# homenc/HElib

Hardware: AMD Instinct MI355X
Metric: ctxt_x_ctxt_mults_per_sec_incl_relinearize (higher is better)
Workload: dtype u64; 1 GPU; BGV m=32768 p=65537 bits=950 (L=16x60b, K=6x56b, 6 small primes, D=3): Ctxt::multiplyBy on FRESH ciphertexts = multLowLvl (bringToSet x2 + tensorProduct) + reLinearize (dropSmallAndSpecialPrimes + key switch), benchmarks/bgv_basic.cpp:144-165; added noise MEASURED as in the reference (device canonical-embedding norms, read back lazily); the loop is driven by the C++17 host (libhelib_amd_host.so); ; batch_per_gpu=128, pairs_all_ranks=128

## Files before the change

### helib_amd/build.py

```python
import os
import shutil
import subprocess
import sys
from concurrent.futures import ThreadPoolExecutor

HERE = os.path.dirname(os.path.abspath(__file__))
CSRC = os.path.join(HERE, "csrc")
LIBDIR = os.path.join(HERE, "lib")
SO = os.path.join(LIBDIR, "libhelib_amd.so")
UNITS = [("ntt_kernels.hip", ["-DHX_NTT_ONLY=13", "-DHX_NTT_PART=1"], "ntt_kernels_13.o"),
         ("ntt_kernels.hip", ["-DHX_NTT_ONLY=14", "-DHX_NTT_PART=1"], "ntt_kernels_14.o"),
         ("ntt_kernels.hip", ["-DHX_NTT_ONLY=15", "-DHX_NTT_PART=1"], "ntt_kernels_15.o"),
         ("ntt_kernels.hip", ["-DHX_NTT_ONLY=13", "-DHX_NTT_PART=2"], "ntt_kslast_13.o"),
         ("ntt_kernels.hip", ["-DHX_NTT_ONLY=14", "-DHX_NTT_PART=2"], "ntt_kslast_14.o"),
         ("ntt_kernels.hip", ["-DHX_NTT_ONLY=15", "-DHX_NTT_PART=2"], "ntt_kslast_15.o"), ("ntt_dispatch.hip", [], "ntt_dispatch.o"),
         ("conv_kernels.hip", [], "conv_kernels.o"), ("pfa_kernels.hip", [], "pfa_kernels.o"), ("rns_mfma_kernels.hip", [], "rns_mfma_kernels.o"),
         ("ckks_slots.hip", [], "ckks_slots.o"), ("bgv_slots.hip", [], "bgv_slots.o"), ("bgv_crt.hip", [], "bgv_crt.o"),
         ("bgv_gf.hip", [], "bgv_gf.o"), ("bgv_gf_linalg.hip", [], "bgv_gf_linalg.o"),
         ("linalg.hip", [], "linalg.o"),
         ("engine.hip", [], "engine.o")]
SOURCES = sorted({u[0] for u in UNITS})
HEADERS = ["ntt_core.h", "dev_common.h", "rns_kernels.h", "rns_types.h", "hostmath.h", "conv_core.h", "bluestein.h", "norm_kernels.h",
           "prg_kernels.h", "arena.h", "prof.h", "conv_dev.h", "ntt_kernel_util.h", "norm_r16.h", "fft_lds.h", "work_map.h",
           os.path.join("..", "..", "include", "helib_amd.h")]
UNIT_HEADERS = {"pfa_kernels.hip": ["pfa_core.h", "pfa_dev.h"], "rns_mfma_kernels.hip": ["mfma_ext.h", "rns_mfma_dev.h"],
                "engine.hip": ["pfa_core.h", "pfa_dev.h", "switches.h", "mfma_ext.h", "rns_mfma_dev.h", "ckks_bridge.h"],
                "ckks_slots.hip": ["ckks_slots.h", "ckks_bridge.h"], "bgv_slots.hip": ["bgv_slots.h", "bgv_encode.h", "ckks_bridge.h"],
                "bgv_crt.hip": ["bgv_slots.h", "bgv_encode.h", "bgv_crt.h", "ckks_bridge.h"],
                "bgv_gf.hip": ["bgv_slots.h", "bgv_encode.h", "bgv_crt.h", "bgv_gf.h", "bgv_gf_tail.h", "ckks_bridge.h"],
                "bgv_gf_linalg.hip": ["bgv_slots.h", "bgv_encode.h", "bgv_crt.h", "bgv_gf.h", "bgv_gf_linalg.h", "bgv_gf_tail.h",
                                      "gather_map.h", "ckks_bridge.h"],
                "linalg.hip": ["ckks_bridge.h"]}
FLAGS = ["--offload-arch=gfx950", "-O3", "-std=c++17", "-fPIC", "-Wno-unused-value",
         "-Wno-pass-failed"]


def hipcc():
    for cand in (shutil.which("hipcc"), "/opt/rocm/bin/hipcc"):
        if cand and os.path.exists(cand):
            return cand
    raise RuntimeError("hipcc not found: the MI355X engine cannot be built")


def _stale(target, deps):
    if not os.path.exists(target):
        return True
    t = os.path.getmtime(target)
    return any(os.path.getmtime(d) > t for d in deps if os.path.exists(d))


def build(force=False, extra_flags=(), verbose=False):
    os.makedirs(LIBDIR, exist_ok=True)
    deps = [os.path.join(CSRC, h) for h in HEADERS] + [os.path.abspath(__file__)]
    cc = hipcc()
    objs, jobs = [], []
    for s, unit_flags, o in UNITS:
        src = os.path.join(CSRC, s)
        obj = os.path.join(LIBDIR, o)
        objs.append(obj)
        if force or _stale(obj, deps + [src] + [os.path.join(CSRC, h) for h in UNIT_HEADERS.get(s, [])]):
            jobs.append([cc, *FLAGS, *unit_flags, *extra_flags, "-c", src, "-o", obj])

    def run(cmd):
        if verbose:
            print(" ".join(cmd), file=sys.stderr)
        subprocess.check_call(cmd)

    if jobs:
        with ThreadPoolExecutor(max_workers=len(jobs)) as ex:
            list(ex.map(run, jobs))
    if jobs or force or _stale(SO, objs):
        run([cc, "--offload-arch=gfx950", "-shared", "-fPIC", "-o", SO, *objs])
    build_host(force=force, verbose=verbose)
    return SO


HOST_SO = os.path.join(LIBDIR, "libhelib_amd_host.so")


def build_host(force=False, verbose=False, link_dir=None, link_lib="helib_amd", out=None):
    inc = os.path.join(HERE, "..", "include")
    src = os.path.join(CSRC, "host_session.cpp")
    out = out or HOST_SO
    deps = [src] + [os.path.join(inc, h) for h in os.listdir(inc)]
    if not (force or _stale(out, deps)):
        return out
    cmd = ["g++", "-std=c++17", "-O2", "-fPIC", "-shared", "-Wall", "-I" + inc, src, "-L" + (link_dir or LIBDIR),
           "-l" + link_lib, "-Wl,-rpath," + (link_dir or "$ORIGIN"), "-o", out]
    if verbose:
        print(" ".join(cmd), file=sys.stderr)
    subprocess.check_call(cmd)
    return out


if __name__ == "__main__":
    print(build(force="--force" in sys.argv, verbose=True))
```

### helib_amd/csrc/dev_common.h

```cpp
#pragma once
#include <hip/hip_runtime.h>
#include <stdint.h>

#include "ntt_core.h"

namespace hx {

constexpr int MAX_ROWS = 160;

struct PrimeDev {
  uint64_t q;
  uint64_t q2;
  uint64_t mu;
  uint64_t mu64;
  uint32_t k;
  uint32_t proth;
  uint64_t mu63;
  uint64_t tw_fwd_off;
  uint64_t tw_inv_off;
  uint64_t r2;
  uint64_t half_t1, half_t1p, half_t1m;
};

struct RowMap {
// ... 49 lines not shown
}
__device__ __forceinline__ uint64_t ld_stream1(const uint64_t* p)
{
#if defined(HX_NO_NT) || defined(HX_RNS_NO_NT)
  return *p;
#else
  return __builtin_nontemporal_load(p);
#endif
}
__device__ __forceinline__ void st_stream1(uint64_t* p, uint64_t v)
{
#if defined(HX_NO_NT) || defined(HX_RNS_NO_NT)
  *p = v;
#else
  __builtin_nontemporal_store(v, p);
#endif
}
__device__ __forceinline__ void st_stream2(uint64_t* p, ulonglong2 v)
{
#ifdef HX_NO_NT
  *reinterpret_cast<ulonglong2*>(p) = v;
#else
  hx_v2u64 w;
  w.x = v.x;
  w.y = v.y;
  __builtin_nontemporal_store(w, reinterpret_cast<hx_v2u64*>(p));
#endif
}
#endif

struct TensorSrc {
  const uint64_t* a0;
  const uint64_t* a1;
  const uint64_t* b0;
  const uint64_t* b1;
};
constexpr int MD_MAXPOLY = 8;
struct PolyBases {
  uint64_t* d[MD_MAXPOLY];
  int n;
};
__host__ __device__ inline uint64_t* poly_base(const PolyBases& p, unsigned i)
{
  uint64_t* r = p.d[0];
  r = i == 1 ? p.d[1] : r;
  r = i == 2 ? p.d[2] : r;
  r = i == 3 ? p.d[3] : r;
  r = i == 4 ? p.d[4] : r;
  r = i == 5 ? p.d[5] : r;
  r = i == 6 ? p.d[6] : r;
  r = i == 7 ? p.d[7] : r;
  return r;
}
struct RowMap2 {
  uint16_t p[MAX_ROWS];
  uint16_t brow[MAX_ROWS];
};
struct RowScalars {
  uint64_t c[MAX_ROWS];
  uint64_t cp[MAX_ROWS];
};

constexpr int KS_MAXD = 8;
struct KsFix {
  int64_t owner;
  TW pinv[KS_MAXD];
  TW pscale;
};
struct KsLastPlan {
  uint16_t fd[MAX_ROWS];
};
struct KsLastArgs {
  const uint64_t* dig_in;
  const uint64_t* dig_ev;
  const uint64_t* kb;
  const uint64_t* ka;
  uint64_t* out0;
  uint64_t* out1;
  const uint64_t* own_src;
  const uint64_t* acc0;
  const uint64_t* acc1;
  const KsFix* fix;
  int nall, wrows, batch, scale_parts;
};

typedef unsigned __int128 u128;

#define HX_RO __attribute__((address_space(4)))
typedef const HX_RO uint64_t* ro_u64;
typedef const HX_RO uint32_t* ro_u32;
typedef const HX_RO double* ro_f64;
typedef const HX_RO TW* ro_tw;
template <class T>
__host__ __device__ inline const HX_RO T* as_ro(const T* p)
{
  return (const HX_RO T*)(uintptr_t)p;
}
__device__ __forceinline__ TW ld_tw(ro_tw p, size_t i)
{
  ro_u64 w = (ro_u64)p;
  TW t;
  t.w = w[2 * i];
  t.wp = w[2 * i + 1];
  return t;
}

__device__ __forceinline__ uint64_t add_mod(uint64_t a, uint64_t b, uint64_t q)
{
  uint64_t s = a + b;
  return s >= q ? s - q : s;
}
__device__ __forceinline__ uint64_t sub_mod(uint64_t a, uint64_t b, uint64_t q)
{
  return a >= b ? a - b : a + q - b;
}
__device__ __forceinline__ uint64_t neg_mod(uint64_t a, uint64_t q) { return a ? q - a : 0; }

__device__ __forceinline__ uint64_t mul_mod(uint64_t a, uint64_t b, uint64_t q, uint64_t mu,
                                            uint32_t k)
{
  u128 x = (u128)a * b;
  uint64_t xs = (uint64_t)(x >> (k - 1));
  uint64_t qh = (uint64_t)(((u128)xs * mu) >> (k + 1));
  uint64_t r = (uint64_t)x - qh * q;
  r = r >= q ? r - q : r;
  return r >= q ? r - q : r;
}
__device__ __forceinline__ uint64_t red128_wide(u128 x, uint64_t q, uint64_t mu, uint32_t k)
{
  uint64_t xs = (uint64_t)(x >> (k - 1));
  uint64_t qh = (uint64_t)(((u128)xs * mu) >> (k + 1));
  uint64_t r = (uint64_t)x - qh * q;
  uint64_t q8 = q << 3, q4 = q << 2, q2 = q << 1;
  r = r >= q8 ? r - q8 : r;
  r = r >= q4 ? r - q4 : r;
  r = r >= q2 ? r - q2 : r;
  return r >= q ? r - q : r;
}
__device__ __forceinline__ uint64_t red64(uint64_t x, uint64_t q, uint64_t mu64)
{
  uint64_t qh = __umul64hi(x, mu64);
  uint64_t r = x - qh * q;
  return r >= q ? r - q : r;
}
__device__ __forceinline__ uint64_t mul_shoup(uint64_t x, uint64_t c, uint64_t cp, uint64_t q)
{
  uint64_t h = __umul64hi(x, cp);
  uint64_t r = x * c - h * q;
  return r >= q ? r - q : r;
}

}
```

### helib_amd/csrc/engine.hip

```cpp
#include <hip/hip_runtime.h>

#include <cstdarg>
#include <cstdio>
#include <cstdlib>
#include <cstring>
#include <algorithm>
#include <chrono>
#include <map>
#include <mutex>
#include <string>
#include <unordered_set>
#include <vector>

#include "../../include/helib_amd.h"
#include "arena.h"
#include "prof.h"
#include "switches.h"
#include "dev_common.h"
#include "hostmath.h"
#include "bluestein.h"
#include "pfa_dev.h"
#include "rns_kernels.h"
#include "mfma_ext.h"
#include "rns_mfma_dev.h"
// ... 4317 lines not shown
  for (int r = 0; r < nall; r++) {
    int wr = find_row(W->row_idx, all[r]);
    if (wr < 0)
      return fail(HX_ERR_PRIMESET, "key-switching matrix is not defined on the operand's primes");
    map.p[r] = (uint16_t)all[r];
    map.brow[r] = (uint16_t)wr;
  }
  size_t rw = (size_t)batch * c->phim;
  int lazy = W->ndig <= 8 ? 1 : 0;
  for (int r : all)
    if (hxh::bitlen(c->primes[r].q) > 60)
      lazy = 0;
  const hx::KsFix* d_fix = nullptr;
  if (own_src || ts)
    CHK(ks_fix_table(c, all, *owner, *digit_primes, &d_fix));
#define HX_KS_LAUNCH(ND)                                                                                           \
  HX_LAUNCH(hx::keyswitch_kernel<ND>, ew_grid(rw, nall), dim3(256), 0, c->stream, dig, W->d_b, W->d_a, out0, out1,  \
            map, ndig, nall, (int)W->row_idx.size(), batch, c->phim, accumulate_rows, c->d_primes, own_src, d_fix,  \
            lazy, d_fix ? t0s : nullptr, d_fix ? t1s : nullptr,                                                    \
            ts ? *ts : hx::TensorSrc{nullptr, nullptr, nullptr, nullptr})
  switch (ndig) {
    case 2: HX_KS_LAUNCH(2); break;
    case 3: HX_KS_LAUNCH(3); break;
    case 4: HX_KS_LAUNCH(4); break;
    default: HX_KS_LAUNCH(0); break;
  }
#undef HX_KS_LAUNCH
  HIPCHK(hipGetLastError());
  return HX_OK;
}

static std::vector<int> ks_last_digit(const std::vector<int>& owner, int ndig)
{
  std::vector<int> fd(owner.size());
  for (size_t r = 0; r < owner.size(); r++)
    fd[r] = owner[r] == ndig - 1 ? ndig - 2 : ndig - 1;
  return fd;
}
static bool ks_last_ok(const hx_ctx* c, const hx_ksk* W, const std::vector<int>& all, const std::vector<int>& owner, int L,
                       int ndig)
{
  if (c->sw.no_ks_last_fuse || !c->pow2 || c->logn < 13 || c->logn > 15 || ndig < 2 || ndig > 4 || W->ndig > 8 ||
      (int)all.size() > MAX_ROWS)
    return false;
  for (size_t r = 0; r < all.size(); r++) {
    const uint64_t q = c->primes[(size_t)all[r]].q;
    if (hxh::bitlen(q) > 60 || (q >> 32) == 0 || (owner[r] >= 0) != ((int)r < L) || owner[r] >= ndig)
      return false;
  }
  return true;
}
static int keyswitch_last_launch(hx_ctx* c, const uint64_t* dig_in, const uint64_t* dig_ev, const hx_ksk* W,
                                 const std::vector<int>& all, int batch, uint64_t* out0, uint64_t* out1, const uint64_t* own_src,
                                 const std::vector<int>& owner, const std::vector<std::vector<int>>& digit_primes, int ndig,
                                 const uint64_t* t0s, const uint64_t* t1s)
{
  const int nall = (int)all.size();
  RowMap2 map;
  hx::KsLastPlan plan;
  const std::vector<int> fd = ks_last_digit(owner, ndig);
  for (int r = 0; r < nall; r++) {
    int wr = find_row(W->row_idx, all[r]);
    if (wr < 0)
      return fail(HX_ERR_PRIMESET, "key-switching matrix is not defined on the operand's primes");
    map.p[r] = (uint16_t)all[r];
    map.brow[r] = (uint16_t)wr;
    plan.fd[r] = (uint16_t)fd[r];
  }
  hx::KsLastArgs A;
  CHK(ks_fix_table(c, all, owner, digit_primes, &A.fix));
  A.dig_in = dig_in;
  A.dig_ev = dig_ev;
  A.kb = W->d_b;
  A.ka = W->d_a;
  A.out0 = out0;
  A.out1 = out1;
  A.own_src = own_src;
  A.acc0 = t0s ? t0s : out0;
  A.acc1 = t0s ? t1s : out1;
  A.scale_parts = t0s ? 1 : 0;
  A.nall = nall;
  A.wrows = (int)W->row_idx.size();
  A.batch = batch;
  hipError_t e = hx::launch_keyswitch_last_pow2(c->logn, ndig, A, map, plan, c->device, c->d_primes, c->d_tw, c->stream);
  if (e != hipSuccess)
    return fail(HX_ERR_DEVICE, "key-switch launch failed: %s", hipGetErrorString(e));
  return HX_OK;
}

extern "C" int hx_key_switch_digits(const hx_poly* digits, const hx_ksk* W, hx_poly* out0,
                                    hx_poly* out1)
{
  if (!digits || !W || !out0 || !out1)
    return fail(HX_ERR_INVALID, "null argument");
  hx_ctx* c = digits->ctx;
  CTX_ENTER(c);
  const int nall = out0->nrows();
  if (nall == 0 || out1->prime_idx != out0->prime_idx || out0->batch != digits->batch ||
      out1->batch != digits->batch)
    return fail(HX_ERR_PRIMESET, "Ctxt::addPart: ctxt has primes not in part");
  if (digits->nrows() % nall != 0 || digits->nrows() / nall > W->ndig || digits->nrows() == 0)
    return fail(HX_ERR_INVALID, "W must have as many columns as there are digits");
  const int ndig = digits->nrows() / nall;
  for (int d = 0; d < ndig; d++)
    for (int r = 0; r < nall; r++)
      if (digits->prime_idx[(size_t)d * nall + r] != out0->prime_idx[r])
        return fail(HX_ERR_PRIMESET, "digit rows do not match the ciphertext's primes");
  OWN(out0);
  OWN(out1);
  return keyswitch_launch(c, digits->d, W, out0->prime_idx, digits->batch, out0->d, out1->d, nall,
                          nullptr, nullptr, nullptr, ndig);
}

static int relin_core(hx_ctx* c, const uint64_t* t2e, const std::vector<int>& own,
                      const std::vector<int>& all, const hx_ksk* W, const int* dig_idx,
                      const int* dig_off, int ndig, int batch, uint64_t* out0, uint64_t* out1,
                      const uint64_t* t0s = nullptr, const uint64_t* t1s = nullptr, const hx::TensorSrc* ts = nullptr)
{
  const int L = (int)own.size(), nall = (int)all.size();
  const size_t rw = (size_t)batch * c->phim;
  CHK(ensure_scratch(c, 2, (size_t)L * rw));
  if (ts) {
    NttRows nr;
    for (int r = 0; r < L; r++) {
      nr.row[r] = (uint16_t)r;
      nr.prime[r] = (uint16_t)own[r];
    }
    hipError_t e = hx::launch_ntt_inv_mul_pow2(c->logn, ts->a1, ts->b1, c->scratch[2], nr, L, batch, c->d_primes,
                                               c->d_tw, c->stream);
    if (e != hipSuccess)
      return fail(HX_ERR_DEVICE, "NTT launch failed: %s", hipGetErrorString(e));
  } else {
    std::vector<std::pair<int, int>> rows;
    for (int r = 0; r < L; r++)
      rows.emplace_back(r, own[r]);
    CHK(ntt_list(c, t2e, c->scratch[2], rows, batch, true));
  }
  CHK(ensure_scratch(c, 1, (size_t)ndig * nall * rw));
  std::vector<int> owner;
  {
    int rc = break_digits_fused(c, c->scratch[2], own, dig_idx, dig_off, ndig, all, c->scratch[1],
                                rw, &owner, digits_lazy_ok(c));
    if (rc == HX_ERR_UNSUPPORTED)
      rc = break_digits_coef(c, c->scratch[2], own, dig_idx, dig_off, ndig, all, c->scratch[1], rw,
                             false, &owner);
    if (rc != HX_OK)
      return rc;
  }
  uint64_t* digits_eval = c->scratch[1];
  const bool fuse_last = !ts && ks_last_ok(c, W, all, owner, L, ndig);
  const std::vector<int> fd = fuse_last ? ks_last_digit(owner, ndig) : std::vector<int>(nall, -1);
  {
    std::vector<std::pair<int, int>> rows;
    for (int d = 0; d < ndig; d++)
      for (int r = 0; r < nall; r++)
        if (owner[r] != d && fd[r] != d)
          rows.emplace_back(d * nall + r, all[r]);
    if (c->pow2 && c->logn == 15 && c->sw.half15) {
      CHK(ensure_scratch(c, 10, (size_t)ndig * nall * rw));
      digits_eval = c->scratch[10];
    }
    CHK(ntt_list(c, c->scratch[1], digits_eval, rows, batch, false, true));
  }
  std::vector<std::vector<int>> dprimes(ndig);
  for (int d = 0; d < ndig; d++)
    dprimes[d].assign(dig_idx + dig_off[d], dig_idx + dig_off[d + 1]);
// ... 293 lines not shown
```

### helib_amd/csrc/ntt_kernels.hip

```cpp
#include <cstdlib>
#include "dev_common.h"
#include "prof.h"

#include "ntt_kernel_util.h"

#ifdef HX_NTT_ONLY
#define HX_SFX2(n, s) n##_L##s
#define HX_SFX1(n, s) HX_SFX2(n, s)
#define HX_ENTRY(n) HX_SFX1(n, HX_NTT_ONLY)
#else
#define HX_ENTRY(n) n
#endif
#if !defined(HX_NTT_ONLY) || HX_NTT_ONLY == 13
#define HX_SZ_13(...) case 13: return __VA_ARGS__;
#else
#define HX_SZ_13(...)
#endif
#if !defined(HX_NTT_ONLY) || HX_NTT_ONLY == 14
#define HX_SZ_14(...) case 14: return __VA_ARGS__;
#else
#define HX_SZ_14(...)
#endif
#if !defined(HX_NTT_ONLY) || HX_NTT_ONLY == 15
#define HX_SZ_15(...) case 15: return __VA_ARGS__;
#else
#define HX_SZ_15(...)
#endif
#define HX_SZ(N, ...) HX_SZ_##N(__VA_ARGS__)

namespace hx {

typedef int v4i32 __attribute__((ext_vector_type(4)));
typedef int v2i32 __attribute__((ext_vector_type(2)));
__device__ v2i32 hx_buffer_load_v2(v4i32 rsrc, int voffset, int soffset,
                                   int aux) __asm("llvm.amdgcn.raw.buffer.load.v2i32");
__device__ void hx_buffer_store_v2(v2i32 data, v4i32 rsrc, int voffset, int soffset,
                                   int aux) __asm("llvm.amdgcn.raw.buffer.store.v2i32");

#ifdef HX_NO_NT
#define HX_NT 0
#define HX_NT_ASM ""
#else
#define HX_NT 2
#define HX_NT_ASM " nt"
#endif

__device__ v4i32 hx_buffer_load_v4(v4i32 rsrc, int voffset, int soffset,
                                   int aux) __asm("llvm.amdgcn.raw.buffer.load.v4i32");

__device__ __forceinline__ v4i32 make_rsrc(const uint64_t* row, unsigned bytes)
{
  uint64_t a = (uint64_t)row;
  v4i32 r;
  r.x = __builtin_amdgcn_readfirstlane((int)(uint32_t)a);
  r.y = __builtin_amdgcn_readfirstlane((int)(uint32_t)(a >> 32));
  r.z = (int)bytes;
  r.w = 0x00020000;
  return r;
}
struct BufTw {
  v4i32 r;
  const TW* p;
  __device__ explicit BufTw(const TW* tw) : r(make_rsrc(reinterpret_cast<const uint64_t*>(tw), 0xfffffff0u)), p(tw) {}
};
__device__ __forceinline__ TW tw_uni(const BufTw& t, unsigned i) { return t.p[i]; }
__device__ __forceinline__ TW tw_vec(const BufTw& t, unsigned base, unsigned lane, unsigned off, uint32_t dep)
{
  int vo = (int)(lane * 16u);
  asm volatile("" : "+v"(vo) : "v"(dep));
  const v4i32 x = hx_buffer_load_v4(t.r, vo, (int)((base + off) * 16u), 0);
  TW w;
  w.w = ((uint64_t)(uint32_t)x.y << 32) | (uint32_t)x.x;
  w.wp = ((uint64_t)(uint32_t)x.w << 32) | (uint32_t)x.z;
  return w;
}

template <int LB>
struct BufIOT {
  static constexpr int LOAD_BOUND = LB;
#ifndef HX_DIGITS_LB8
  template <class AR>
  static constexpr int load_bound() { return (LB == 8 && AR::PROTH) ? 2 : LB; }
#endif
  static constexpr bool LAZY_STORE = false;
  static constexpr bool PIPELINED = false;
  struct StorePrefetch {};
  v4i32 rin, rout;
// ... 567 lines not shown
      pinned_wait<(g > 0 ? CPG : 0) + (more ? 8 : 0)>(wb[g & 1]);
      static_for<0, CPG>([&](auto J) {
        constexpr int j = decltype(J)::value;
        if constexpr (P1)
          one(std::integral_constant<int, g * CPG + j>{}, wb[g & 1][4 * j], wb[g & 1][4 * j + 1], wb[g & 1][4 * j + 2],
              wb[g & 1][4 * j + 3]);
        else
          one(std::integral_constant<int, g * CPG + j>{}, wb[g & 1][2 * j], wb[g & 1][2 * j + 1], 0, 0);
      });
      HX_SCHED_FENCE();
    });
  }
  template <int LOGN, class AR, int B, bool EST>
  __device__ __forceinline__ void store_all(unsigned tid, uint64_t (&v)[32], const QC& qc, StorePrefetch&) const
  {
    if (part == 1)
      store_part<LOGN, AR, B, EST, true>(tid, v, qc);
    else
      store_part<LOGN, AR, B, EST, false>(tid, v, qc);
  }
  __device__ __forceinline__ void put(unsigned tid, unsigned c, uint64_t o) const
  {
    asm volatile("buffer_store_dwordx2 %0, %1, %2, %3 offen" HX_NT_ASM
                 :
                 : "v"(o), "v"((int)(tid * 8u)), "s"(ro), "s"((int)(c * 8u))
                 : "memory");
  }
  __device__ __forceinline__ TW last_tw(TW def, int) const { return def; }
  __device__ __forceinline__ TWM last_tw(TWM def, int) const { return def; }
};
template <int LOGN, bool PLAIN>
__global__ void __launch_bounds__(Geo<LOGN>::T, HX_NTT_MINWAVES(LOGN))
ntt_moddown_apply_tensor_kernel(TensorSrc T, PolyBases outs, NttRows rows, int nkeep, int batch, ModDownApply A,
                                const PrimeDev* __restrict__ primes, const TW* __restrict__ tw_arena)
{
  extern __shared__ __attribute__((aligned(16))) uint32_t lds[];
  const MdWork Wk = md_work(blockIdx.x, (unsigned)nkeep, 3u * (unsigned)batch);
  if (!Wk.active)
    return;
  const unsigned ri = Wk.ri, pb = Wk.pb;
#ifdef HX_TENSOR_PARTS_APART
  const int b = (int)(pb % (unsigned)batch);
  const unsigned pi = pb / (unsigned)batch;
#else
  const int b = (int)(pb / 3u);
  const unsigned pi = pb % 3u;
#endif
  const PrimeDev* pd = primes + uniform_u16(rows.prime, ri);
  const size_t N = Geo<LOGN>::N;
  const ModDownRow R = A.rows[ri];
  uint64_t* odata = poly_base(outs, pi);
  const size_t eoff = ((size_t)pi * batch + b) * N;
  const uint64_t* xrow = PLAIN ? A.delta + (size_t)pi * (size_t)A.delta_poly_stride + ((size_t)ri * batch + b) * N
                               : A.xs + eoff;
  const ModDownTensorIO<PLAIN> io(xrow, PLAIN ? nullptr : A.S + eoff, R, T, pi,
                                  ((size_t)uniform_u16(rows.row, ri) * batch + b) * N, R.mode != 2,
                                  odata + ((size_t)R.out_row * batch + b) * N, (unsigned)N * 8u, pd);
  ntt_body<LOGN, false>(lds, io, tw_arena + pd->tw_fwd_off, pd);
}

template <int LOGN, bool INV, int LB = 1>
__global__ void __launch_bounds__(Geo<LOGN>::T, HX_NTT_MINWAVES(LOGN))
ntt_row_kernel(const uint64_t* in, uint64_t* out, NttRows rows, int batch,
               const PrimeDev* __restrict__ primes, const TW* __restrict__ tw_arena)
{
  extern __shared__ __attribute__((aligned(16))) uint32_t lds[];
  const unsigned wid = xcd_remap(blockIdx.x, gridDim.x);
  const unsigned ri = wid / (unsigned)batch;
  const int b = (int)(wid % (unsigned)batch);
  const int row = (int)uniform_u16(rows.row, ri);
  const PrimeDev* pd = primes + uniform_u16(rows.prime, ri);
  const size_t roff = ((size_t)row * batch + b) * (size_t)Geo<LOGN>::N;
  const TW* tw = tw_arena + (INV ? pd->tw_inv_off : pd->tw_fwd_off);

#ifdef HX_NTT_PTRIO
  const PtrIO io{in + roff, out + roff};
#else
  const BufIOT<LB> io(in + roff, out + roff, (unsigned)Geo<LOGN>::N * 8u);
#endif
  ntt_body<LOGN, INV>(lds, io, tw, pd);
}

#if !defined(HX_NTT_PART) || HX_NTT_PART == 2
template <int ND>
struct KsLastIO {
  static constexpr int LOAD_BOUND = 8;
#ifndef HX_DIGITS_LB8
  template <class AR>
  static constexpr int load_bound() { return AR::PROTH ? 2 : 8; }
#endif
  static constexpr bool LAZY_STORE = true;
  static constexpr bool PIPELINED = false;
  static constexpr int DEPTH = ND <= 2 ? 2 : 1;
  static constexpr bool SPLIT = ND >= 4;
  struct StorePrefetch {};
  v4i32 rin;
  const KsLastArgs& A;
  unsigned row, b, brow, fd;
  int owner;
  uint64_t q, mu63, mu64;
  uint32_t k;
  TW ps;
  TW pinv[ND - 1];
  __device__ KsLastIO(const KsLastArgs& A_, unsigned row_, unsigned b_, unsigned brow_, unsigned fd_, unsigned bytes,
                      const PrimeDev* pd)
      : rin(make_rsrc(A_.dig_in + (((size_t)fd_ * (size_t)A_.nall + row_) * (size_t)A_.batch + b_) * (size_t)(bytes / 8u), bytes)),
        A(A_), row(row_), b(b_), brow(brow_), fd(fd_), q(pd->q), mu63(pd->mu63), mu64(pd->mu64), k(pd->k)
  {
    ro_u64 fw = as_ro(reinterpret_cast<const uint64_t*>(A_.fix + row_));
    constexpr unsigned PINV = offsetof(KsFix, pinv) / 8u, PSC = offsetof(KsFix, pscale) / 8u;
    owner = (int)(int64_t)fw[0];
    ps.w = A_.scale_parts ? fw[PSC] : 1;
    ps.wp = A_.scale_parts ? fw[PSC + 1] : mu64;
#pragma unroll
    for (int e = 0; e < ND - 1; e++) {
      const bool in = e < owner;
      pinv[e].w = in ? fw[PINV + 2 * e] : 1;
      pinv[e].wp = in ? fw[PINV + 2 * e + 1] : mu64;
    }
  }
  __device__ __forceinline__ uint64_t load(unsigned tid, unsigned c) const
  {
    v2i32 r = hx_buffer_load_v2(rin, (int)(tid * 8u), (int)(c * 8u), HX_NT);
    return ((uint64_t)(uint32_t)r.y << 32) | (uint32_t)r.x;
  }
  template <int LOGN>
  __device__ __forceinline__ void store_prefetch(unsigned, StorePrefetch&) const {}
  template <bool NT>
  static __device__ __forceinline__ uint64_t ld_pinned(const v4i32& r, unsigned tid, int soff)
  {
    uint64_t x;
    if constexpr (NT)
      asm volatile("buffer_load_dwordx2 %0, %1, %2, %3 offen" HX_NT_ASM : "=v"(x) : "v"((int)(tid * 8u)), "s"(r), "s"(soff) : "memory");
    else
      asm volatile("buffer_load_dwordx2 %0, %1, %2, %3 offen" : "=v"(x) : "v"((int)(tid * 8u)), "s"(r), "s"(soff) : "memory");
    return x;
  }
  static __device__ __forceinline__ void put(const v4i32& r, unsigned tid, unsigned c, uint64_t o)
  {
    asm volatile("buffer_store_dwordx2 %0, %1, %2, %3 offen" HX_NT_ASM : : "v"(o), "v"((int)(tid * 8u)), "s"(r), "s"((int)(c * 8u)) : "memory");
  }
#define HX_KV(i) "+v"(x[i])
#define HX_KS_WAIT(NW, ...)                                                                \
  template <int N>                                                                         \
  static __device__ __forceinline__ void pinned_wait(uint64_t (&x)[NW])                    \
  {                                                                                        \
    asm volatile("s_waitcnt vmcnt(%" #NW ")" : __VA_ARGS__ : "n"(N) : "memory");           \
  }
  HX_KS_WAIT(4, HX_KV(0), HX_KV(1), HX_KV(2), HX_KV(3))
  HX_KS_WAIT(5, HX_KV(0), HX_KV(1), HX_KV(2), HX_KV(3), HX_KV(4))
  HX_KS_WAIT(7, HX_KV(0), HX_KV(1), HX_KV(2), HX_KV(3), HX_KV(4), HX_KV(5), HX_KV(6))
  HX_KS_WAIT(9, HX_KV(0), HX_KV(1), HX_KV(2), HX_KV(3), HX_KV(4), HX_KV(5), HX_KV(6), HX_KV(7), HX_KV(8))
  HX_KS_WAIT(8, HX_KV(0), HX_KV(1), HX_KV(2), HX_KV(3), HX_KV(4), HX_KV(5), HX_KV(6), HX_KV(7))
  HX_KS_WAIT(10, HX_KV(0), HX_KV(1), HX_KV(2), HX_KV(3), HX_KV(4), HX_KV(5), HX_KV(6), HX_KV(7), HX_KV(8), HX_KV(9))
  HX_KS_WAIT(11, HX_KV(0), HX_KV(1), HX_KV(2), HX_KV(3), HX_KV(4), HX_KV(5), HX_KV(6), HX_KV(7), HX_KV(8), HX_KV(9), HX_KV(10))
  HX_KS_WAIT(13, HX_KV(0), HX_KV(1), HX_KV(2), HX_KV(3), HX_KV(4), HX_KV(5), HX_KV(6), HX_KV(7), HX_KV(8), HX_KV(9), HX_KV(10),
             HX_KV(11), HX_KV(12))
#undef HX_KS_WAIT
#undef HX_KV
  template <int LOGN, class AR, int B, bool OWNED>
  __device__ __forceinline__ void store_rows(unsigned tid, uint64_t (&v)[32], const QC& qc) const
  {
    constexpr int NMEM = OWNED ? ND - 2 : ND - 1, NACC = OWNED ? 3 : 0, NW = NMEM + NACC + (SPLIT ? ND : 2 * ND);
    constexpr int KB0 = NMEM + NACC, KA0 = KB0 + ND;
    constexpr size_t N = Geo<LOGN>::N;
    constexpr unsigned bytes = (unsigned)N * 8u;
    const size_t eoff = ((size_t)row * (size_t)A.batch + b) * N;
    const size_t dstride = (size_t)A.nall * (size_t)A.batch * N;
    const unsigned kstride = (unsigned)A.wrows * bytes;
    v4i32 rm[NMEM > 0 ? NMEM : 1];
    int kd[ND];
#pragma unroll
    for (int s = 0; s < NMEM; s++) {
      const unsigned d = (OWNED && s >= owner) ? (unsigned)s + 1u : (unsigned)s;
      rm[s] = make_rsrc(A.dig_ev + (size_t)d * dstride + eoff, bytes);
      kd[s] = (int)(d * kstride);
    }
    kd[NMEM] = (int)(fd * kstride);
    if constexpr (OWNED)
      kd[NMEM + 1] = (int)((unsigned)owner * kstride);
    const v4i32 rkb = make_rsrc(A.kb + (size_t)brow * N, (unsigned)(ND - 1) * kstride + bytes);
    const v4i32 rka = make_rsrc(A.ka + (size_t)brow * N, (unsigned)(ND - 1) * kstride + bytes);
    const v4i32 ro0 = make_rsrc(A.out0 + eoff, bytes), ro1 = make_rsrc(A.out1 + eoff, bytes);
    const v4i32 rown = make_rsrc(OWNED ? A.own_src + eoff : A.out0 + eoff, bytes);
    const v4i32 ra0 = make_rsrc(OWNED ? A.acc0 + eoff : A.out0 + eoff, bytes);
    const v4i32 ra1 = make_rsrc(OWNED ? (A.acc1 ? A.acc1 : A.acc0) + eoff : A.out0 + eoff, bytes);
    const uint64_t m1 = A.acc1 ? ~(uint64_t)0 : 0;
    uint32_t cm[NMEM > 0 ? NMEM : 1];
#pragma unroll
    for (int s = 0; s < NMEM; s++)
      cm[s] = s < owner ? ~0u : 0u;
    const uint32_t cmf = (owner == ND - 1) ? ~0u : 0u;
    auto masked = [](uint64_t x, uint32_t m) { return ((uint64_t)((uint32_t)(x >> 32) & m) << 32) | ((uint32_t)x & m); };
    auto request = [&](auto I, uint64_t (&w)[NW]) {
      constexpr int i = decltype(I)::value;
      const int c8 = (int)(eval_const<LOGN>(i) * 8u);
      static_for<0, NMEM>([&](auto S) { w[decltype(S)::value] = ld_pinned<true>(rm[decltype(S)::value], tid, c8); });
      if constexpr (OWNED) {
        w[NMEM] = ld_pinned<true>(rown, tid, c8);
        w[NMEM + 1] = ld_pinned<true>(ra0, tid, c8);
        w[NMEM + 2] = ld_pinned<true>(ra1, tid, c8);
      }
      static_for<0, ND>([&](auto S) { w[KB0 + decltype(S)::value] = ld_pinned<false>(rkb, tid, kd[decltype(S)::value] + c8); });
      if constexpr (!SPLIT)
        static_for<0, ND>([&](auto S) { w[KA0 + decltype(S)::value] = ld_pinned<false>(rka, tid, kd[decltype(S)::value] + c8); });
    };
    uint64_t wb[DEPTH][NW];
    uint64_t k2[ND];
    request(std::integral_constant<int, 0>{}, wb[0]);
    static_for<0, 32>([&](auto II) {
      constexpr int i = decltype(II)::value;
      constexpr bool more = i + 1 < 32;
      uint64_t(&w)[NW] = wb[DEPTH == 2 ? (i & 1) : 0];
      if constexpr (DEPTH == 2) {
        if constexpr (more)
          request(std::integral_constant<int, i + 1>{}, wb[(i + 1) & 1]);
        pinned_wait<(i > 0 ? 2 : 0) + (more ? NW : 0)>(w);
      } else {
        pinned_wait<(i > 0 ? (SPLIT ? 1 : 2) : 0)>(w);
      }
      const uint64_t xf = norm_from<B, true>(v[i], qc);
      const unsigned c = eval_const<LOGN>(i);
      uint64_t x[ND];
      static_for<0, NMEM>([&](auto S) { x[decltype(S)::value] = w[decltype(S)::value]; });
      x[NMEM] = xf;
      u128 s0 = 0, s1 = 0;
      if constexpr (OWNED) {
        uint64_t own = w[NMEM];
        static_for<0, NMEM>([&](auto S) {
          constexpr int s = decltype(S)::value;
          own = mul_shoup(own + q - masked(w[s], cm[s]), pinv[s].w, pinv[s].wp, q);
        });
        x[NMEM + 1] = mul_shoup(own + q - masked(xf, cmf), pinv[ND - 2].w, pinv[ND - 2].wp, q);
        s0 = mul_shoup(w[NMEM + 1], ps.w, ps.wp, q);
        s1 = mul_shoup(w[NMEM + 2], ps.w, ps.wp, q) & m1;
      }
      static_for<0, ND>([&](auto S) { s0 += (u128)x[decltype(S)::value] * w[KB0 + decltype(S)::value]; });
      if constexpr (SPLIT) {
        const int c8 = (int)(c * 8u);
        static_for<0, ND>([&](auto S) { k2[decltype(S)::value] = ld_pinned<false>(rka, tid, kd[decltype(S)::value] + c8); });
        put(ro0, tid, c, tensor_red128(s0, q, mu63, k));
        pinned_wait<1>(k2);
        static_for<0, ND>([&](auto S) { s1 += (u128)x[decltype(S)::value] * k2[decltype(S)::value]; });
        if constexpr (more)
          request(std::integral_constant<int, i + 1>{}, wb[0]);
        put(ro1, tid, c, tensor_red128(s1, q, mu63, k));
      } else {
        static_for<0, ND>([&](auto S) { s1 += (u128)x[decltype(S)::value] * w[KA0 + decltype(S)::value]; });
        if constexpr (DEPTH == 1 && more)
          request(std::integral_constant<int, i + 1>{}, wb[0]);
        put(ro0, tid, c, tensor_red128(s0, q, mu63, k));
        put(ro1, tid, c, tensor_red128(s1, q, mu63, k));
      }
      HX_SCHED_FENCE();
    });
  }
  template <int LOGN, class AR, int B, bool EST>
  __device__ __forceinline__ void store_all(unsigned tid, uint64_t (&v)[32], const QC& qc, StorePrefetch&) const
  {
    if constexpr (EST) {
      if (owner >= 0)
        store_rows<LOGN, AR, B, true>(tid, v, qc);
      else
        store_rows<LOGN, AR, B, false>(tid, v, qc);
    }
  }
  __device__ __forceinline__ TW last_tw(TW def, int) const { return def; }
  __device__ __forceinline__ TWM last_tw(TWM def, int) const { return def; }
};
template <int LOGN, int ND>
__global__ void __launch_bounds__(Geo<LOGN>::T, HX_NTT_MINWAVES(LOGN))
ntt_keyswitch_last_kernel(KsLastArgs A, RowMap2 map, KsLastPlan plan, const PrimeDev* __restrict__ primes,
                          const TW* __restrict__ tw_arena)
{
  extern __shared__ __attribute__((aligned(16))) uint32_t lds[];
  const KsWork W = ks_last_work(blockIdx.x, (unsigned)A.nall, (unsigned)A.batch);
  const PrimeDev* pd = primes + uniform_u16(map.p, W.row);
  const KsLastIO<ND> io(A, W.row, W.b, uniform_u16(map.brow, W.row), uniform_u16(plan.fd, W.row), (unsigned)Geo<LOGN>::N * 8u, pd);
  ntt_body<LOGN, false>(lds, io, tw_arena + pd->tw_fwd_off, pd);
}
template <int LOGN, int ND>
static hipError_t launch_ks_last(const KsLastArgs& A, const RowMap2& map, const KsLastPlan& plan, int device,
                                 const PrimeDev* primes, const TW* tw_arena, hipStream_t st)
{
  constexpr size_t lds_bytes = (size_t)Geo<LOGN>::LDS_WORDS * 4;
  hipError_t e = hxp::dyn_lds((const void*)ntt_keyswitch_last_kernel<LOGN, ND>, (int)lds_bytes, device);
  if (e != hipSuccess)
    return e;
  HX_LAUNCH((ntt_keyswitch_last_kernel<LOGN, ND>), dim3((unsigned)A.nall * (unsigned)A.batch), dim3(Geo<LOGN>::T), lds_bytes,
            st, A, map, plan, primes, tw_arena);
  return hipGetLastError();
}
template <int LOGN>
static hipError_t launch_ks_last_nd(int nd, const KsLastArgs& A, const RowMap2& map, const KsLastPlan& plan, int device,
                                    const PrimeDev* primes, const TW* tw_arena, hipStream_t st)
{
  switch (nd) {
    case 2: return launch_ks_last<LOGN, 2>(A, map, plan, device, primes, tw_arena, st);
    case 3: return launch_ks_last<LOGN, 3>(A, map, plan, device, primes, tw_arena, st);
    case 4: return launch_ks_last<LOGN, 4>(A, map, plan, device, primes, tw_arena, st);
  }
  return hipErrorInvalidValue;
}
hipError_t HX_ENTRY(launch_keyswitch_last_pow2)(int logn, int nd, const KsLastArgs& A, const RowMap2& map, const KsLastPlan& plan,
                                                int device, const PrimeDev* primes, const TW* tw_arena, hipStream_t st)
{
  switch (logn) {
    HX_SZ(13, launch_ks_last_nd<13>(nd, A, map, plan, device, primes, tw_arena, st))
    HX_SZ(14, launch_ks_last_nd<14>(nd, A, map, plan, device, primes, tw_arena, st))
    HX_SZ(15, launch_ks_last_nd<15>(nd, A, map, plan, device, primes, tw_arena, st))
  }
  return hipErrorInvalidValue;
}
#endif

#if !defined(HX_NTT_PART) || HX_NTT_PART == 1
template <bool PROTH>
struct MulLoadIO {
  static constexpr int LOAD_BOUND = 1;
  static constexpr bool LAZY_STORE = false;
  static constexpr bool PIPELINED = false;
  template <class AR>
  static constexpr int inv_load_bound() { return PROTH ? 2 : 1; }
  struct StorePrefetch {};
  v4i32 ra, rb, ro;
  uint64_t q, mu63, r2;
  uint32_t k;
  __device__ MulLoadIO(const uint64_t* a_row, const uint64_t* b_row, uint64_t* o_row, unsigned bytes, const PrimeDev* pd)
      : ra(make_rsrc(a_row, bytes)), rb(make_rsrc(b_row, bytes)), ro(make_rsrc(o_row, bytes)), q(pd->q), mu63(pd->mu63),
        r2(pd->r2), k(pd->k)
  {
  }
  __device__ __forceinline__ uint64_t load(unsigned tid, unsigned c) const
  {
    const v2i32 x = hx_buffer_load_v2(ra, (int)(tid * 8u), (int)(c * 8u), HX_NT);
    const v2i32 y = hx_buffer_load_v2(rb, (int)(tid * 8u), (int)(c * 8u), HX_NT);
    const uint64_t a = ((uint64_t)(uint32_t)x.y << 32) | (uint32_t)x.x, b = ((uint64_t)(uint32_t)y.y << 32) | (uint32_t)y.x;
    const u128 p = (u128)a * b;
    if constexpr (PROTH)
      return mont_redc128((uint64_t)p, (uint64_t)(p >> 64), make_qc(q, 0));
    else
      return tensor_red128(p, q, mu63, k);
  }
  __device__ __forceinline__ void store(unsigned tid, unsigned c, uint64_t v) const
  {
    v2i32 d;
    d.x = (int)(uint32_t)v;
    d.y = (int)(uint32_t)(v >> 32);
    hx_buffer_store_v2(d, ro, (int)(tid * 8u), (int)(c * 8u), HX_NT);
  }
  __device__ __forceinline__ TW last_tw(TW def, int) const { return def; }
  __device__ __forceinline__ TWM last_tw(TWM def, int) const
  {
    if constexpr (PROTH) {
      const QC qc = make_qc(q, 0);
      return csub(mont_mul(def, r2, qc), q);
    } else {
      return def;
    }
  }
};
template <int LOGN>
__global__ void __launch_bounds__(Geo<LOGN>::T, HX_NTT_MINWAVES(LOGN))
ntt_inv_mul_kernel(const uint64_t* a, const uint64_t* b, uint64_t* out, NttRows rows, int batch,
                   const PrimeDev* __restrict__ primes, const TW* __restrict__ tw_arena)
{
  extern __shared__ __attribute__((aligned(16))) uint32_t lds[];
  const unsigned wid = xcd_remap(blockIdx.x, gridDim.x);
  const unsigned ri = wid / (unsigned)batch;
  const int bb = (int)(wid % (unsigned)batch);
  const int row = (int)uniform_u16(rows.row, ri);
  const PrimeDev* pd = primes + uniform_u16(rows.prime, ri);
  const size_t N = Geo<LOGN>::N;
  const size_t roff = ((size_t)row * batch + bb) * N, ooff = ((size_t)ri * batch + bb) * N;
  const QC qc = make_qc(pd->q, pd->mu64);
  const TW* tw = tw_arena + pd->tw_inv_off;
#ifndef HX_NO_PROTH
  if (pd->proth) {
#ifndef HX_INVMUL_BARRETT
    const MulLoadIO<true> io(a + roff, b + roff, out + ooff, (unsigned)N * 8u, pd);
#else
    const MulLoadIO<false> io(a + roff, b + roff, out + ooff, (unsigned)N * 8u, pd);
// ... 458 lines not shown
```

### helib_amd/csrc/switches.h

```cpp
#pragma once
#include <cstdlib>

namespace hxs {

struct Switches {
  bool no_hps = false;
  double hps_eps = 1.0 / (double)(1u << 30);
  int hps_min_n = 9;
  int brk_hps_min_n = 5;
  bool no_lazy_rns = false;
  bool no_fast_break = false;
  bool no_fast_extend = false;
  bool no_proth_rns = false;
  bool no_wide_extend = false;
  bool no_mfma_ext = false;
  int mfma_min_n = 9;
  bool no_mask_split = false;
  int brk_lds_pad_rows = 0;
  bool no_tensor_multi = false;
  bool no_mulrelin_fuse = false;
  bool no_ks_last_fuse = false;
  bool half15 = false;
  bool no_proth = false;
  bool blue_old = false;
  bool no_pfa = false;
  bool pfa_no_rem = false;
  bool norm_async = false;
  bool norm_old = false;
  bool norm_plain = false;
  bool norm_memcpy = false;
  int wait_poll_us = 2000;
  bool arena_trace = false;
};

inline Switches read()
{
  Switches s;
  auto on = [](const char* name) { return std::getenv(name) != nullptr; };
  s.no_hps = on("HX_NO_HPS");
  if (const char* e = std::getenv("HX_HPS_EPS"))
    s.hps_eps = std::atof(e);
  if (const char* e = std::getenv("HX_HPS_MIN_N"))
    s.hps_min_n = s.brk_hps_min_n = std::atoi(e);
  if (const char* e = std::getenv("HX_BRK_HPS_MIN_N"))
    s.brk_hps_min_n = std::atoi(e);
  s.no_lazy_rns = on("HX_NO_LAZY_RNS");
  s.no_fast_break = on("HX_NO_FAST_BREAK");
  s.no_fast_extend = on("HX_NO_FAST_EXTEND");
  s.no_proth_rns = on("HX_NO_PROTH_RNS");
  s.no_wide_extend = on("HX_NO_WIDE_EXTEND");
  s.no_mfma_ext = on("HX_NO_MFMA_EXT") || s.no_wide_extend;
  if (const char* e = std::getenv("HX_MFMA_MIN_N"))
    s.mfma_min_n = std::atoi(e);
  s.no_mask_split = on("HX_NO_MASK_SPLIT");
  if (const char* e = std::getenv("HX_BRK_LDS_PAD"))
    s.brk_lds_pad_rows = std::atoi(e);
  s.half15 = on("HX_HALF15");
  s.no_tensor_multi = on("HX_NO_TENSOR_MULTI");
  s.no_mulrelin_fuse = on("HX_NO_MULRELIN_FUSE");
  s.no_ks_last_fuse = on("HX_NO_KS_LAST_FUSE");
  s.no_proth = on("HX_NO_PROTH");
  s.blue_old = on("HX_BLUE_OLD");
  s.no_pfa = on("HX_NO_PFA") || s.blue_old;
  s.pfa_no_rem = on("HX_PFA_NO_REM");
  s.norm_async = on("HX_NORM_ASYNC");
  s.norm_old = on("HX_NORM_OLD");
  s.norm_plain = on("HX_NORM_PLAIN");
  s.norm_memcpy = on("HX_NORM_MEMCPY");
  if (const char* e = std::getenv("HX_WAIT_POLL_US"))
    s.wait_poll_us = std::atoi(e);
  s.arena_trace = on("HX_ARENA_TRACE");
  return s;
}

}
```

Before: 44230 mult/s.

## Stage key-switch streamed operands through idle LDS with buffer-to-LDS loads

After: 44380 mult/s, median of 6. Within noise of the previous version (+0.3%).

```diff
diff --git a/helib_amd/build.py b/helib_amd/build.py
--- a/helib_amd/build.py
+++ b/helib_amd/build.py
@@ -21,7 +21,7 @@
          ("engine.hip", [], "engine.o")]
 SOURCES = sorted({u[0] for u in UNITS})
 HEADERS = ["ntt_core.h", "dev_common.h", "rns_kernels.h", "rns_types.h", "hostmath.h", "conv_core.h", "bluestein.h", "norm_kernels.h",
-           "prg_kernels.h", "arena.h", "prof.h", "conv_dev.h", "ntt_kernel_util.h", "norm_r16.h", "fft_lds.h", "work_map.h",
+           "prg_kernels.h", "arena.h", "prof.h", "conv_dev.h", "ntt_kernel_util.h", "norm_r16.h", "fft_lds.h", "work_map.h", "lds_stage.h",
            os.path.join("..", "..", "include", "helib_amd.h")]
 UNIT_HEADERS = {"pfa_kernels.hip": ["pfa_core.h", "pfa_dev.h"], "rns_mfma_kernels.hip": ["mfma_ext.h", "rns_mfma_dev.h"],
                 "engine.hip": ["pfa_core.h", "pfa_dev.h", "switches.h", "mfma_ext.h", "rns_mfma_dev.h", "ckks_bridge.h"],
diff --git a/helib_amd/csrc/dev_common.h b/helib_amd/csrc/dev_common.h
--- a/helib_amd/csrc/dev_common.h
+++ b/helib_amd/csrc/dev_common.h
@@ -155,6 +155,7 @@
   const uint64_t* acc1;
   const KsFix* fix;
   int nall, wrows, batch, scale_parts;
+  int lds_stage;
 };
 
 typedef unsigned __int128 u128;
diff --git a/helib_amd/csrc/engine.hip b/helib_amd/csrc/engine.hip
--- a/helib_amd/csrc/engine.hip
+++ b/helib_amd/csrc/engine.hip
@@ -4423,6 +4423,7 @@
   A.nall = nall;
   A.wrows = (int)W->row_idx.size();
   A.batch = batch;
+  A.lds_stage = (ndig == 3 && !c->sw.no_ks_lds_stage) ? 1 : 0;
   hipError_t e = hx::launch_keyswitch_last_pow2(c->logn, ndig, A, map, plan, c->device, c->d_primes, c->d_tw, c->stream);
   if (e != hipSuccess)
     return fail(HX_ERR_DEVICE, "key-switch launch failed: %s", hipGetErrorString(e));
diff --git a/helib_amd/csrc/lds_stage.h b/helib_amd/csrc/lds_stage.h
--- /dev/null
+++ b/helib_amd/csrc/lds_stage.h
@@ -0,0 +1,37 @@
+#pragma once
+#include "ntt_core.h"
+
+namespace hx {
+
+template <int LOGN>
+struct LdsStage {
+  static constexpr int T = Geo<LOGN>::T;
+  static constexpr int WAVES = T / 64;
+  static constexpr int SLOTS = 4;
+  static constexpr int STAGES = 2;
+  static constexpr int PAIRS = 16;
+  static constexpr unsigned PIECE = 1024;
+  static constexpr unsigned HALF = PIECE / 2;
+  static constexpr unsigned WAVE_BYTES = STAGES * SLOTS * PIECE;
+  static constexpr unsigned BYTES = WAVES * WAVE_BYTES;
+  static constexpr int DIST = LOGN == 13 ? 8 : 16;
+  static constexpr unsigned PAIR_WORDS = T;
+
+  static HXD constexpr int first(int p) { return LOGN == 13 ? (p & 7) + ((p >> 3) << 4) : p; }
+  static HXD constexpr int coef(int k) { return first(k >> 1) + (k & 1) * DIST; }
+
+  static HXD unsigned src_off(unsigned wave, unsigned lane)
+  {
+    return wave * 512u + (lane & 31u) * 16u + (lane >> 5) * (PAIR_WORDS * 8u);
+  }
+  static HXD constexpr unsigned wave_base(unsigned wave) { return wave * WAVE_BYTES; }
+  static HXD constexpr unsigned piece_off(unsigned stage, unsigned slot) { return (stage * SLOTS + slot) * PIECE; }
+  static HXD constexpr unsigned read_off(unsigned stage, unsigned slot, unsigned half, unsigned lane)
+  {
+    return piece_off(stage, slot) + half * HALF + lane * 8u;
+  }
+
+  static_assert(BYTES <= (unsigned)Geo<LOGN>::LDS_WORDS * 4u, "the stage fits the idle transpose LDS");
+};
+
+}
diff --git a/helib_amd/csrc/ntt_kernels.hip b/helib_amd/csrc/ntt_kernels.hip
--- a/helib_amd/csrc/ntt_kernels.hip
+++ b/helib_amd/csrc/ntt_kernels.hip
@@ -3,6 +3,7 @@
 #include "prof.h"
 
 #include "ntt_kernel_util.h"
+#include "lds_stage.h"
 
 #ifdef HX_NTT_ONLY
 #define HX_SFX2(n, s) n##_L##s
@@ -736,8 +737,9 @@
 }
 
 #if !defined(HX_NTT_PART) || HX_NTT_PART == 2
-template <int ND>
+template <int ND, bool STAGE = false>
 struct KsLastIO {
+  static_assert(!STAGE || ND == 3, "the stage holds the four streamed words of D = 3");
   static constexpr int LOAD_BOUND = 8;
 #ifndef HX_DIGITS_LB8
   template <class AR>
@@ -751,15 +753,16 @@
   v4i32 rin;
   const KsLastArgs& A;
   unsigned row, b, brow, fd;
+  unsigned lds0;
   int owner;
   uint64_t q, mu63, mu64;
   uint32_t k;
   TW ps;
   TW pinv[ND - 1];
   __device__ KsLastIO(const KsLastArgs& A_, unsigned row_, unsigned b_, unsigned brow_, unsigned fd_, unsigned bytes,
-                      const PrimeDev* pd)
+                      const PrimeDev* pd, unsigned lds0_)
       : rin(make_rsrc(A_.dig_in + (((size_t)fd_ * (size_t)A_.nall + row_) * (size_t)A_.batch + b_) * (size_t)(bytes / 8u), bytes)),
-        A(A_), row(row_), b(b_), brow(brow_), fd(fd_), q(pd->q), mu63(pd->mu63), mu64(pd->mu64), k(pd->k)
+        A(A_), row(row_), b(b_), brow(brow_), fd(fd_), lds0(lds0_), q(pd->q), mu63(pd->mu63), mu64(pd->mu64), k(pd->k)
   {
     ro_u64 fw = as_ro(reinterpret_cast<const uint64_t*>(A_.fix + row_));
     constexpr unsigned PINV = offsetof(KsFix, pinv) / 8u, PSC = offsetof(KsFix, pscale) / 8u;
@@ -779,7 +782,73 @@
     return ((uint64_t)(uint32_t)r.y << 32) | (uint32_t)r.x;
   }
   template <int LOGN>
-  __device__ __forceinline__ void store_prefetch(unsigned, StorePrefetch&) const {}
+  __device__ __forceinline__ void store_prefetch(unsigned tid, StorePrefetch&) const
+  {
+    if constexpr (STAGE) {
+      asm volatile("s_waitcnt lgkmcnt(0)" ::: "memory");
+      __builtin_amdgcn_s_barrier();
+      if (owner >= 0)
+        stage_first<LOGN, true>(tid);
+      else
+        stage_first<LOGN, false>(tid);
+    }
+  }
+  template <bool OWNED>
+  static constexpr int nstream() { return OWNED ? ND + 1 : ND - 1; }
+  template <int LOGN, bool OWNED>
+  __device__ __forceinline__ void stream_rsrc(v4i32 (&rs)[nstream<OWNED>()]) const
+  {
+    constexpr int NMEM = OWNED ? ND - 2 : ND - 1;
+    constexpr size_t N = Geo<LOGN>::N;
+    constexpr unsigned bytes = (unsigned)N * 8u;
+    const size_t eoff = ((size_t)row * (size_t)A.batch + b) * N;
+    const size_t dstride = (size_t)A.nall * (size_t)A.batch * N;
+#pragma unroll
+    for (int s = 0; s < NMEM; s++) {
+      const unsigned d = (OWNED && s >= owner) ? (unsigned)s + 1u : (unsigned)s;
+      rs[s] = make_rsrc(A.dig_ev + (size_t)d * dstride + eoff, bytes);
+    }
+    if constexpr (OWNED) {
+      rs[NMEM] = make_rsrc(A.own_src + eoff, bytes);
+      rs[NMEM + 1] = make_rsrc(A.acc0 + eoff, bytes);
+      rs[NMEM + 2] = make_rsrc((A.acc1 ? A.acc1 : A.acc0) + eoff, bytes);
+    }
+  }
+  static __device__ __forceinline__ void ld_stage(const v4i32& r, int voff, unsigned ldst, int soff)
+  {
+    unsigned keep;
+    asm volatile("s_mov_b32 %0, m0\n\ts_mov_b32 m0, %3\n\ts_nop 0\n\tbuffer_load_dwordx4 %1, %2, %4 offen" HX_NT_ASM " lds\n\ts_mov_b32 m0, %0"
+                 : "=&s"(keep)
+                 : "v"(voff), "s"(r), "s"(ldst), "s"(soff)
+                 : "memory");
+  }
+  template <int LOGN, bool OWNED, int P>
+  __device__ __forceinline__ void stage_pair(const v4i32 (&rs)[nstream<OWNED>()], int voff, unsigned wbase) const
+  {
+    using St = LdsStage<LOGN>;
+    static_assert(nstream<OWNED>() <= St::SLOTS && P < St::PAIRS, "stage");
+    const int c8 = (int)(eval_const<LOGN>(St::first(P)) * 8u);
+    static_for<0, nstream<OWNED>()>([&](auto S) {
+      constexpr int s = decltype(S)::value;
+      ld_stage(rs[s], voff, wbase + St::piece_off(P & 1, s), c8);
+    });
+  }
+  template <int LOGN, bool OWNED>
+  __device__ __forceinline__ void stage_first(unsigned tid) const
+  {
+    using St = LdsStage<LOGN>;
+    v4i32 rs[nstream<OWNED>()];
+    stream_rsrc<LOGN, OWNED>(rs);
+    const unsigned wv = wave_index();
+    stage_pair<LOGN, OWNED, 0>(rs, (int)St::src_off(wv, tid & 63u), lds0 + St::wave_base(wv));
+  }
+  static __device__ __forceinline__ uint64_t ld_lds(unsigned addr, int off)
+  {
+    uint64_t x;
+    asm volatile("ds_read_b64 %0, %1 offset:%2" : "=v"(x) : "v"(addr), "n"(off) : "memory");
+    return x;
+  }
+  static __device__ __forceinline__ void lds_landed(uint64_t& x) { asm volatile("" : "+v"(x)); }
   template <bool NT>
   static __device__ __forceinline__ uint64_t ld_pinned(const v4i32& r, unsigned tid, int soff)
   {
@@ -803,6 +872,7 @@
   }
   HX_KS_WAIT(4, HX_KV(0), HX_KV(1), HX_KV(2), HX_KV(3))
   HX_KS_WAIT(5, HX_KV(0), HX_KV(1), HX_KV(2), HX_KV(3), HX_KV(4))
+  HX_KS_WAIT(6, HX_KV(0), HX_KV(1), HX_KV(2), HX_KV(3), HX_KV(4), HX_KV(5))
   HX_KS_WAIT(7, HX_KV(0), HX_KV(1), HX_KV(2), HX_KV(3), HX_KV(4), HX_KV(5), HX_KV(6))
   HX_KS_WAIT(9, HX_KV(0), HX_KV(1), HX_KV(2), HX_KV(3), HX_KV(4), HX_KV(5), HX_KV(6), HX_KV(7), HX_KV(8))
   HX_KS_WAIT(8, HX_KV(0), HX_KV(1), HX_KV(2), HX_KV(3), HX_KV(4), HX_KV(5), HX_KV(6), HX_KV(7))
@@ -815,6 +885,10 @@
   template <int LOGN, class AR, int B, bool OWNED>
   __device__ __forceinline__ void store_rows(unsigned tid, uint64_t (&v)[32], const QC& qc) const
   {
+    if constexpr (STAGE) {
+      store_rows_staged<LOGN, AR, B, OWNED>(tid, v, qc);
+      return;
+    }
     constexpr int NMEM = OWNED ? ND - 2 : ND - 1, NACC = OWNED ? 3 : 0, NW = NMEM + NACC + (SPLIT ? ND : 2 * ND);
     constexpr int KB0 = NMEM + NACC, KA0 = KB0 + ND;
     constexpr size_t N = Geo<LOGN>::N;
@@ -909,6 +983,85 @@
       HX_SCHED_FENCE();
     });
   }
+  template <int LOGN, class AR, int B, bool OWNED>
+  __device__ __forceinline__ void store_rows_staged(unsigned tid, uint64_t (&v)[32], const QC& qc) const
+  {
+    using St = LdsStage<LOGN>;
+    constexpr int NMEM = OWNED ? ND - 2 : ND - 1, NS = nstream<OWNED>(), NK = 2 * ND;
+    constexpr size_t N = Geo<LOGN>::N;
+    constexpr unsigned bytes = (unsigned)N * 8u;
+    const size_t eoff = ((size_t)row * (size_t)A.batch + b) * N;
+    const unsigned kstride = (unsigned)A.wrows * bytes;
+    v4i32 rs[NS];
+    stream_rsrc<LOGN, OWNED>(rs);
+    int kd[ND];
+#pragma unroll
+    for (int s = 0; s < NMEM; s++)
+      kd[s] = (int)(((OWNED && s >= owner) ? (unsigned)s + 1u : (unsigned)s) * kstride);
+    kd[NMEM] = (int)(fd * kstride);
+    if constexpr (OWNED)
+      kd[NMEM + 1] = (int)((unsigned)owner * kstride);
+    const v4i32 rkb = make_rsrc(A.kb + (size_t)brow * N, (unsigned)(ND - 1) * kstride + bytes);
+    const v4i32 rka = make_rsrc(A.ka + (size_t)brow * N, (unsigned)(ND - 1) * kstride + bytes);
+    const v4i32 ro0 = make_rsrc(A.out0 + eoff, bytes), ro1 = make_rsrc(A.out1 + eoff, bytes);
+    const uint64_t m1 = A.acc1 ? ~(uint64_t)0 : 0;
+    uint32_t cm[NMEM > 0 ? NMEM : 1];
+#pragma unroll
+    for (int s = 0; s < NMEM; s++)
+      cm[s] = s < owner ? ~0u : 0u;
+    const uint32_t cmf = (owner == ND - 1) ? ~0u : 0u;
+    auto masked = [](uint64_t x, uint32_t m) { return ((uint64_t)((uint32_t)(x >> 32) & m) << 32) | ((uint32_t)x & m); };
+    const unsigned wv = wave_index(), lane = tid & 63u;
+    const unsigned wbase = lds0 + St::wave_base(wv);
+    const int voff = (int)St::src_off(wv, lane);
+    const unsigned raddr = wbase + lane * 8u;
+    uint64_t w[NK];
+    auto keys = [&](auto K) {
+      const int c8 = (int)(eval_const<LOGN>(St::coef(decltype(K)::value)) * 8u);
+      static_for<0, ND>([&](auto S) { w[decltype(S)::value] = ld_pinned<false>(rkb, tid, kd[decltype(S)::value] + c8); });
+      static_for<0, ND>([&](auto S) { w[ND + decltype(S)::value] = ld_pinned<false>(rka, tid, kd[decltype(S)::value] + c8); });
+    };
+    keys(std::integral_constant<int, 0>{});
+    stage_pair<LOGN, OWNED, 1>(rs, voff, wbase);
+    static_for<0, 32>([&](auto KK) {
+      constexpr int k = decltype(KK)::value, i = St::coef(k), p = k >> 1, h = k & 1;
+      constexpr bool more = k + 1 < 32;
+      constexpr bool staged_before = k == 0 || (k >= 2 && h == 0 && p + 1 < St::PAIRS);
+      pinned_wait<(k > 0 ? 2 : 0) + (staged_before ? NS : 0)>(w);
+      uint64_t sw[NS];
+      static_for<0, NS>([&](auto S) {
+        constexpr int s = decltype(S)::value;
+        sw[s] = ld_lds(raddr, (int)St::read_off(p & 1, s, h, 0));
+      });
+      asm volatile("s_waitcnt lgkmcnt(0)" ::: "memory");
+      static_for<0, NS>([&](auto S) { lds_landed(sw[decltype(S)::value]); });
+      const uint64_t xf = norm_from<B, true>(v[i], qc);
+      const unsigned c = eval_const<LOGN>(i);
+      uint64_t x[ND];
+      static_for<0, NMEM>([&](auto S) { x[decltype(S)::value] = sw[decltype(S)::value]; });
+      x[NMEM] = xf;
+      u128 s0 = 0, s1 = 0;
+      if constexpr (OWNED) {
+        uint64_t own = sw[NMEM];
+        static_for<0, NMEM>([&](auto S) {
+          constexpr int s = decltype(S)::value;
+          own = mul_shoup(own + q - masked(sw[s], cm[s]), pinv[s].w, pinv[s].wp, q);
+        });
+        x[NMEM + 1] = mul_shoup(own + q - masked(xf, cmf), pinv[ND - 2].w, pinv[ND - 2].wp, q);
+        s0 = mul_shoup(sw[NMEM + 1], ps.w, ps.wp, q);
+        s1 = mul_shoup(sw[NMEM + 2], ps.w, ps.wp, q) & m1;
+      }
+      static_for<0, ND>([&](auto S) { s0 += (u128)x[decltype(S)::value] * w[decltype(S)::value]; });
+      static_for<0, ND>([&](auto S) { s1 += (u128)x[decltype(S)::value] * w[ND + decltype(S)::value]; });
+      if constexpr (more)
+        keys(std::integral_constant<int, k + 1>{});
+      if constexpr (h == 1 && p + 2 < St::PAIRS)
+        stage_pair<LOGN, OWNED, p + 2>(rs, voff, wbase);
+      put(ro0, tid, c, tensor_red128(s0, q, mu63, this->k));
+      put(ro1, tid, c, tensor_red128(s1, q, mu63, this->k));
+      HX_SCHED_FENCE();
+    });
+  }
   template <int LOGN, class AR, int B, bool EST>
   __device__ __forceinline__ void store_all(unsigned tid, uint64_t (&v)[32], const QC& qc, StorePrefetch&) const
   {
@@ -922,7 +1075,7 @@
   __device__ __forceinline__ TW last_tw(TW def, int) const { return def; }
   __device__ __forceinline__ TWM last_tw(TWM def, int) const { return def; }
 };
-template <int LOGN, int ND>
+template <int LOGN, int ND, bool STAGE>
 __global__ void __launch_bounds__(Geo<LOGN>::T, HX_NTT_MINWAVES(LOGN))
 ntt_keyswitch_last_kernel(KsLastArgs A, RowMap2 map, KsLastPlan plan, const PrimeDev* __restrict__ primes,
                           const TW* __restrict__ tw_arena)
@@ -930,18 +1083,19 @@
   extern __shared__ __attribute__((aligned(16))) uint32_t lds[];
   const KsWork W = ks_last_work(blockIdx.x, (unsigned)A.nall, (unsigned)A.batch);
   const PrimeDev* pd = primes + uniform_u16(map.p, W.row);
-  const KsLastIO<ND> io(A, W.row, W.b, uniform_u16(map.brow, W.row), uniform_u16(plan.fd, W.row), (unsigned)Geo<LOGN>::N * 8u, pd);
+  const KsLastIO<ND, STAGE> io(A, W.row, W.b, uniform_u16(map.brow, W.row), uniform_u16(plan.fd, W.row), (unsigned)Geo<LOGN>::N * 8u, pd,
+                               (unsigned)(uintptr_t)(__attribute__((address_space(3))) uint32_t*)lds);
   ntt_body<LOGN, false>(lds, io, tw_arena + pd->tw_fwd_off, pd);
 }
-template <int LOGN, int ND>
+template <int LOGN, int ND, bool STAGE = false>
 static hipError_t launch_ks_last(const KsLastArgs& A, const RowMap2& map, const KsLastPlan& plan, int device,
                                  const PrimeDev* primes, const TW* tw_arena, hipStream_t st)
 {
   constexpr size_t lds_bytes = (size_t)Geo<LOGN>::LDS_WORDS * 4;
-  hipError_t e = hxp::dyn_lds((const void*)ntt_keyswitch_last_kernel<LOGN, ND>, (int)lds_bytes, device);
+  hipError_t e = hxp::dyn_lds((const void*)ntt_keyswitch_last_kernel<LOGN, ND, STAGE>, (int)lds_bytes, device);
   if (e != hipSuccess)
     return e;
-  HX_LAUNCH((ntt_keyswitch_last_kernel<LOGN, ND>), dim3((unsigned)A.nall * (unsigned)A.batch), dim3(Geo<LOGN>::T), lds_bytes,
+  HX_LAUNCH((ntt_keyswitch_last_kernel<LOGN, ND, STAGE>), dim3((unsigned)A.nall * (unsigned)A.batch), dim3(Geo<LOGN>::T), lds_bytes,
             st, A, map, plan, primes, tw_arena);
   return hipGetLastError();
 }
@@ -951,7 +1105,9 @@
 {
   switch (nd) {
     case 2: return launch_ks_last<LOGN, 2>(A, map, plan, device, primes, tw_arena, st);
-    case 3: return launch_ks_last<LOGN, 3>(A, map, plan, device, primes, tw_arena, st);
+    case 3:
+      return A.lds_stage ? launch_ks_last<LOGN, 3, true>(A, map, plan, device, primes, tw_arena, st)
+                         : launch_ks_last<LOGN, 3>(A, map, plan, device, primes, tw_arena, st);
     case 4: return launch_ks_last<LOGN, 4>(A, map, plan, device, primes, tw_arena, st);
   }
   return hipErrorInvalidValue;
diff --git a/helib_amd/csrc/switches.h b/helib_amd/csrc/switches.h
--- a/helib_amd/csrc/switches.h
+++ b/helib_amd/csrc/switches.h
@@ -20,6 +20,7 @@
   bool no_tensor_multi = false;
   bool no_mulrelin_fuse = false;
   bool no_ks_last_fuse = false;
+  bool no_ks_lds_stage = false;
   bool half15 = false;
   bool no_proth = false;
   bool blue_old = false;
@@ -59,6 +60,7 @@
   s.no_tensor_multi = on("HX_NO_TENSOR_MULTI");
   s.no_mulrelin_fuse = on("HX_NO_MULRELIN_FUSE");
   s.no_ks_last_fuse = on("HX_NO_KS_LAST_FUSE");
+  s.no_ks_lds_stage = on("HX_NO_KS_LDS_STAGE");
   s.no_proth = on("HX_NO_PROTH");
   s.blue_old = on("HX_BLUE_OLD");
   s.no_pfa = on("HX_NO_PFA") || s.blue_old;
```
